# jcorsetti/oryon

Hardware: AMD Instinct MI355X
Metric: image-pairs/sec end-to-end (feat+match+reg) @224², C=256; ADD(-S) parity (higher is better)
Workload: dtype f32

## Files before the change

oryon_amd/csrc/pdsc.h:

```cpp
#pragma once
#include <stdlib.h>
#include <map>
#include <string>
#include <vector>
#include "common.h"

namespace oryon {

struct PdscLayer {
    const float *w_pcn, *b_pcn;
    const float *w_qkv, *b_qkv;
    const float *w_m1, *b_m1;
    const float *w_m2, *b_m2;
    const float *w_m3, *b_m3;
    const char *mlp_img;
    const char *mlp_img_p;
    const char *pq_img;
};

constexpr int PDSC_MLP_W1H = 0, PDSC_MLP_W1L = 16384, PDSC_MLP_W2H = 32768, PDSC_MLP_W2L = 40960, PDSC_MLP_W3H = 49152,
              PDSC_MLP_W3L = 65536, PDSC_MLP_IMG_BYTES = 81920;
constexpr int PDSC_PQ_CHUNK_BYTES = 65536, PDSC_PQ_IMG_BYTES = 5 * PDSC_PQ_CHUNK_BYTES;
constexpr int PDSC_KV_KL = 16384, PDSC_KV_VH = 32768, PDSC_KV_VL = 49152, PDSC_KV_TILE_BYTES = 65536;
constexpr int PDSC_AC_BIAS_OFF = PDSC_MLP_IMG_BYTES + 4 * 64 * (128 / 32 * 16 + 2) * 4, PDSC_AC_BIAS_BYTES = 768 * 4;
__host__ __device__ constexpr int pdsc_k_img_elem(int key, int octet) { return (octet * 64 + key) * 8; }
__host__ __device__ constexpr size_t pdsc_g4_index(int n_cap, int row, int quad) { return (size_t)quad * n_cap + row; }

struct PdscModel {
    oryon_pointdsc_config_t cfg;
    float sigma;
    float sigma_d;
    const float *w0, *b0;
    std::vector<PdscLayer> layers;
    const float *w_c1, *b_c1, *w_c2, *b_c2, *w_c3, *b_c3;
};

struct PdscWorkspace {
    float *corr_pos;
    float *feat;
    float *feat1;
    float *qkv;
    float *msg;
    char *kv_img;
    char *kv_img2;
    float *sc;
    float *att_o;
    float *att_ml;
    int att_splits;
    float *h1, *h2;
    float *feat_n;
    float *conf;
    float *seed_key;
    int32_t *seeds;
    int32_t *n_seeds;
    int32_t *knn;
    float *Mmat;
    float *seed_w;
    float *seed_dist;
    float *v_hist;
    int32_t *close_hist;
    float *seed_T;
    float *fitness;
    int32_t *best;
    float *T0;
    int S_cap, k;
};

inline int pdsc_attention_splits(int B, int n_cap)
{
    static const int forced = dev_env_int("ORYON_PDSC_ATT_SPLITS", 0);
    const int blocks = B * (n_cap / 128);
    int ks = forced ? forced : (256 + blocks - 1) / blocks;
    const int tiles = n_cap / 64;
    if (ks > 4) ks = 4;
    if (ks > tiles) ks = tiles;
    return ks < 1 ? 1 : ks;
}

inline int pdsc_seed_cap(const oryon_pointdsc_config_t &cfg, int n_cap)
{
    return (int)((double)n_cap * (double)cfg.ratio) + 1;
}

void pdsc_launch_normalise(const float *feat, int C, int n_cap, int B, const int32_t *n_rows, float *out, hipStream_t st);
int pdsc_run_encoder(const PdscModel &M, const PdscWorkspace &ws, const float *src, const float *tgt, const int32_t *n_rows,
                     int B, int n_cap, hipStream_t st);
int pdsc_run_seeds(const PdscModel &M, const float *src, const float *conf, const int32_t *n_rows, int B, int n_cap, int S_cap,
                   int32_t *seeds, int32_t *n_seeds, float *key_scratch, hipStream_t st);
int pdsc_run_hypotheses(const PdscModel &M, const PdscWorkspace &ws, const float *src, const float *tgt, const float *feat_n,
                        const int32_t *n_rows, const int32_t *seeds, const int32_t *n_seeds, int B, int n_cap, float *seed_T,
                        float *fitness, int32_t *best, float *T_best, uint8_t *labels, hipStream_t st);
int pdsc_run_refine(const PdscModel &M, const float *src, const float *tgt, const int32_t *n_rows, int B, int n_cap,
                    const float *T_in, const int32_t *status_in, const int32_t *n_seeds, float *T_out, int32_t *status_out,
                    hipStream_t st);

constexpr int PDSC_MAX_K = 64, PDSC_MAX_IT = 16;
int pdsc_run_tail(const float *src, const float *tgt, const int32_t *n_rows, const int32_t *n_seeds, int B, int n_cap, int S_cap, int k,
                  int num_iterations, float inlier_thr, const int32_t *knn, const float *Mmat, float *v_hist, int32_t *close_hist,
                  float *seed_T, float *fitness, int32_t *best, float *T_best, uint8_t *labels, hipStream_t st);
int pdsc_run_refine_tau(const float *src, const float *tgt, const int32_t *n_rows, int B, int n_cap, float tau, const float *T_in,
                        const int32_t *status_in, const int32_t *n_seeds, float *T_out, int32_t *status_out, hipStream_t st);

}
```

oryon_amd/csrc/pdsc_blocks.h:

```cpp
#pragma once
#include "common.h"
#include "pdsc.h"
#include "x3.h"

namespace oryon {

constexpr int ATT_Q = 128, ATT_KT = 64;

template <int PIECES, int WAVES, int PER_WAVE = PIECES / WAVES>
__device__ __forceinline__ void dma_pieces(const char *src, char *lds, int wave_u, int lane)
{
    static_assert(PER_WAVE * WAVES >= PIECES, "pieces per wave");
#pragma unroll
    for (int j = 0; j < PER_WAVE; ++j) {
        const int piece = wave_u * PER_WAVE + j;
        if (PER_WAVE * WAVES == PIECES || piece < PIECES)
            __builtin_amdgcn_global_load_lds((const __attribute__((address_space(1))) void *)(src + piece * 1024 + lane * 16),
                                             (__attribute__((address_space(3))) void *)(lds + piece * 1024), 16, 0, 0);
    }
}
template <int WAVES>
__device__ __forceinline__ void dma_mlp_image(const char *img, char *lds, int wave_u, int lane)
{
    dma_pieces<PDSC_MLP_IMG_BYTES / 1024, WAVES>(img, lds, wave_u, lane);
// ... 79 lines not shown
    const float *b;
    __device__ __forceinline__ float4 operator()(int off, int hi) const { return *reinterpret_cast<const float4 *>(b + off + 4 * hi); }
};
struct BiasLds {
    const float *planes;
    __device__ __forceinline__ float4 operator()(int off, int hi) const
    {
        const int q = (off >> 2) + hi;
        return make_float4(planes[q], planes[192 + q], planes[384 + q], planes[576 + q]);
    }
};

template <class Bias>
__device__ __forceinline__ void next_operand(const f32x16 (&acc)[2], const Bias &bias, int off, int hi, f16x8 (&oh)[4], f16x8 (&ol)[4])
{
#pragma unroll
    for (int rb = 0; rb < 2; ++rb)
#pragma unroll
        for (int j = 0; j < 2; ++j) {
            uint4 uh, ul;
            unsigned *ph = &uh.x, *pl = &ul.x;
#pragma unroll
            for (int g2 = 0; g2 < 2; ++g2) {
                const float4 bv = bias(off + rb * 32 + 8 * (2 * j + g2), hi);
                const int r0 = 8 * j + 4 * g2;
                const float v0 = fmaxf(acc[rb][r0] + bv.x, 0.0f), v1 = fmaxf(acc[rb][r0 + 1] + bv.y, 0.0f);
                const float v2 = fmaxf(acc[rb][r0 + 2] + bv.z, 0.0f), v3 = fmaxf(acc[rb][r0 + 3] + bv.w, 0.0f);
                split2(v0, v1, ph[2 * g2], pl[2 * g2]);
                split2(v2, v3, ph[2 * g2 + 1], pl[2 * g2 + 1]);
            }
            oh[rb * 2 + j] = __builtin_bit_cast(f16x8, uh);
            ol[rb * 2 + j] = __builtin_bit_cast(f16x8, ul);
        }
}

__device__ __forceinline__ void load_split_row(const float *row, int hi, f16x8 (&xh)[8], f16x8 (&xl)[8])
{
    const float4 *xp = reinterpret_cast<const float4 *>(row);
    float4 raw[16];
#pragma unroll
    for (int s_ = 0; s_ < 8; ++s_) { raw[2 * s_] = xp[4 * s_ + 2 * hi]; raw[2 * s_ + 1] = xp[4 * s_ + 2 * hi + 1]; }
#pragma unroll
    for (int s_ = 0; s_ < 8; ++s_) {
        uint4 uh, ul;
        split2(raw[2 * s_].x, raw[2 * s_].y, uh.x, ul.x);
        split2(raw[2 * s_].z, raw[2 * s_].w, uh.y, ul.y);
        split2(raw[2 * s_ + 1].x, raw[2 * s_ + 1].y, uh.z, ul.z);
        split2(raw[2 * s_ + 1].z, raw[2 * s_ + 1].w, uh.w, ul.w);
        xh[s_] = __builtin_bit_cast(f16x8, uh);
        xl[s_] = __builtin_bit_cast(f16x8, ul);
    }
}

__device__ __forceinline__ void att8_block_map(int &b, int &qblk)
{
    const int lin = blockIdx.x + gridDim.x * blockIdx.z;
    b = (lin / 8 / (int)gridDim.x) * 8 + (lin & 7);
    qblk = (lin / 8) % (int)gridDim.x;
}
__device__ __forceinline__ void fetch_sc(const float4 *sc_q, bool q_live, int kb, int j0, float4 (&scv)[4])
{
    const float4 *sp = sc_q + (size_t)(j0 / ATT_KT) * 8 * 64 + (size_t)kb * 4 * 64;
#pragma unroll
    for (int v4 = 0; v4 < 4; ++v4) scv[v4] = q_live ? sp[(size_t)v4 * 64] : make_float4(-1.f, -1.f, -1.f, -1.f);
}
__device__ __forceinline__ void read_k(const char *tile, int key, int s_, int hi, f16x8 (&kf)[2])
{
    kf[0] = *reinterpret_cast<const f16x8 *>(reinterpret_cast<const _Float16 *>(tile) + pdsc_k_img_elem(key, 2 * s_ + hi));
    kf[1] = *reinterpret_cast<const f16x8 *>(reinterpret_cast<const _Float16 *>(tile + PDSC_KV_KL) + pdsc_k_img_elem(key, 2 * s_ + hi));
}
__device__ __forceinline__ f16x8 read_v(const char *v_plane, int oct, int ch)
{
    return *reinterpret_cast<const f16x8 *>(reinterpret_cast<const _Float16 *>(v_plane) + ((size_t)oct * 128 + ch) * 8);
}
__device__ __forceinline__ void store_k(char *tile, float4 k, int key, int cc)
{
    uint2 uh, ul;
    split2(k.x, k.y, uh.x, ul.x);
    split2(k.z, k.w, uh.y, ul.y);
    const size_t off = (size_t)pdsc_k_img_elem(key, cc >> 3) * 2 + (cc & 7) * 2;
    *reinterpret_cast<uint2 *>(tile + off) = uh;
    *reinterpret_cast<uint2 *>(tile + PDSC_KV_KL + off) = ul;
}
__device__ __forceinline__ void store_v(char *tile, const f32x16 &acc, float bv, int kb, int ch, int hi)
{
#pragma unroll
    for (int t2 = 0; t2 < 2; ++t2) {
        uint4 uh, ul;
        split2(acc[8 * t2 + 0] + bv, acc[8 * t2 + 1] + bv, uh.x, ul.x);
        split2(acc[8 * t2 + 2] + bv, acc[8 * t2 + 3] + bv, uh.y, ul.y);
        split2(acc[8 * t2 + 4] + bv, acc[8 * t2 + 5] + bv, uh.z, ul.z);
        split2(acc[8 * t2 + 6] + bv, acc[8 * t2 + 7] + bv, uh.w, ul.w);
        const int oct = (kb * 2 + t2) * 2 + hi;
        *reinterpret_cast<uint4 *>(tile + PDSC_KV_VH + ((size_t)oct * 128 + ch) * 16) = uh;
        *reinterpret_cast<uint4 *>(tile + PDSC_KV_VL + ((size_t)oct * 128 + ch) * 16) = ul;
    }
}

}
```

oryon_amd/csrc/pdsc_encoder.hip:

```cpp
#include <stdlib.h>
#include "common.h"
#include "pdsc.h"
#include "pdsc_blocks.h"

namespace oryon {

__global__ __launch_bounds__(256) void pdsc_center_kernel(const float *__restrict__ src, const float *__restrict__ tgt,
                                                           const int32_t *__restrict__ n_rows, int n_cap,
                                                           float *__restrict__ corr_pos )
{
    __shared__ double s_part[4][6];
    __shared__ float s_mean[6];
    const int b = blockIdx.x, t = threadIdx.x, lane = t & 63, wave = t >> 6;
    const int n = n_rows[b];
    const float *s = src + (size_t)b * n_cap * 3, *g = tgt + (size_t)b * n_cap * 3;
    double acc[6] = {0, 0, 0, 0, 0, 0};
    for (int i = t; i < n; i += 256) {
#pragma unroll
        for (int d = 0; d < 3; ++d) { acc[d] += s[3 * i + d]; acc[3 + d] += g[3 * i + d]; }
    }
#pragma unroll
    for (int d = 0; d < 6; ++d) {
        double v = acc[d];
#pragma unroll
// ... 722 lines not shown
#pragma unroll
            for (int j = 0; j < 2; ++j) {
                const f16x8 bh = *reinterpret_cast<const f16x8 *>(Wh + (wn * 64 + j * 32 + l31) * XLD + ko);
                const f16x8 bl = *reinterpret_cast<const f16x8 *>(Wl + (wn * 64 + j * 32 + l31) * XLD + ko);
                acc[j] = __builtin_amdgcn_mfma_f32_32x32x16_f16(ah, bh, acc[j], 0, 0, 0);
                acc[j] = __builtin_amdgcn_mfma_f32_32x32x16_f16(ah, bl, acc[j], 0, 0, 0);
                acc[j] = __builtin_amdgcn_mfma_f32_32x32x16_f16(al, bh, acc[j], 0, 0, 0);
            }
        }
    }
#pragma unroll
    for (int j = 0; j < 2; ++j) {
        const int c = n0 + wn * 64 + j * 32 + l31;
        if (c >= N) continue;
        const float bv = bias ? bias[c] : 0.0f;
#pragma unroll
        for (int r = 0; r < 16; ++r) {
            const int row = m0 + wm * 32 + crow(r, hi);
            float v = acc[j][r] + bv;
            if (RELU) v = v > 0.0f ? v : 0.0f;
            if (RESID) v += R[(size_t)b * r_batch + (size_t)row * ldr + c];
            Y[(size_t)b * y_batch + (size_t)row * ldy + c] = v;
        }
    }
}

template <int WAVES>
__global__ __launch_bounds__(64 * WAVES) void pdsc_mlp3_x3_kernel(const float *__restrict__ msg, const float *__restrict__ resid,
                                                            const char *__restrict__ img, const float *__restrict__ b1,
                                                            const float *__restrict__ b2, const float *__restrict__ b3,
                                                            const int32_t *__restrict__ n_rows, int n_cap, float *__restrict__ out)
{
    constexpr int C = 128;
    extern __shared__ __attribute__((aligned(1024))) char mlp_lds[];
    const int b = blockIdx.y, q0 = blockIdx.x * (32 * WAVES);
    if (q0 >= n_rows[b]) return;
    const int t = threadIdx.x, lane = t & 63, wave = t >> 6, l31 = lane & 31, hi = lane >> 5;
    const int wave_u = __builtin_amdgcn_readfirstlane(wave);
    dma_mlp_image<WAVES>(img, mlp_lds, wave_u, lane);
    const size_t prow = ((size_t)b * n_cap + q0 + wave * 32 + l31) * C;
    f16x8 xh[8], xl[8];
    load_split_row(msg + prow, hi, xh, xl);
    asm volatile("s_waitcnt vmcnt(0)" ::: "memory");
    __syncthreads();
    const Frag256 w1_frag{mlp_lds, l31, hi};
    const Frag128 w23_frag{mlp_lds, l31, hi};
    f32x16 a1[2];
    two_blocks<8, false>(w1_frag, PDSC_MLP_W1H, PDSC_MLP_W1L, 0, xh, xl, a1);
    f16x8 h1h[4], h1l[4];
    next_operand(a1, BiasVector{b1}, 0, hi, h1h, h1l);
    f32x16 a2[2];
    two_blocks<4, false>(w23_frag, PDSC_MLP_W2H, PDSC_MLP_W2L, 0, h1h, h1l, a2);
    f16x8 h2h[4], h2l[4];
    next_operand(a2, BiasVector{b2}, 0, hi, h2h, h2l);
#pragma unroll
    for (int rp = 0; rp < 2; ++rp) {
        float4 rv[2][4];
#pragma unroll
        for (int i = 0; i < 2; ++i)
#pragma unroll
            for (int g = 0; g < 4; ++g) rv[i][g] = *reinterpret_cast<const float4 *>(resid + prow + (2 * rp + i) * 32 + 8 * g + 4 * hi);
        f32x16 a3[2];
        two_blocks<4, false>(w23_frag, PDSC_MLP_W3H, PDSC_MLP_W3L, 2 * rp, h2h, h2l, a3);
#pragma unroll
        for (int i = 0; i < 2; ++i)
#pragma unroll
            for (int g = 0; g < 4; ++g) {
                const int c = (2 * rp + i) * 32 + 8 * g + 4 * hi;
                const float4 bv = *reinterpret_cast<const float4 *>(b3 + c);
                float4 o;
                o.x = a3[i][4 * g + 0] + bv.x + rv[i][g].x;
                o.y = a3[i][4 * g + 1] + bv.y + rv[i][g].y;
                o.z = a3[i][4 * g + 2] + bv.z + rv[i][g].z;
                o.w = a3[i][4 * g + 3] + bv.w + rv[i][g].w;
                *reinterpret_cast<float4 *>(out + prow + c) = o;
            }
    }
}

template <int WAVES>
__global__ __launch_bounds__(64 * WAVES) void pdsc_pcn_qkv_x3_kernel(const float *__restrict__ feat, const char *__restrict__ img,
                                                               const float *__restrict__ bp, const float *__restrict__ bq,
                                                               const int32_t *__restrict__ n_rows, int n_cap, float *__restrict__ feat1,
                                                               float *__restrict__ qkv, char *__restrict__ kv_img, int g4)
{
    constexpr int C = 128, HALF = PDSC_PQ_CHUNK_BYTES / 2;
    extern __shared__ __attribute__((aligned(1024))) char pq_lds[];
    const int b = blockIdx.y, q0 = blockIdx.x * (32 * WAVES);
    if (q0 >= n_rows[b]) return;
    const int t = threadIdx.x, lane = t & 63, wave = t >> 6, l31 = lane & 31, hi = lane >> 5;
    const int wave_u = __builtin_amdgcn_readfirstlane(wave);
    dma_pq_chunk<WAVES>(img, 0, pq_lds, wave_u, lane);
    dma_pq_chunk<WAVES>(img, 1, pq_lds + PDSC_PQ_CHUNK_BYTES, wave_u, lane);
    const size_t prow = (size_t)b * n_cap + q0 + wave * 32 + l31;
    f16x8 xh[8], xl[8];
    load_split_row(feat + prow * C, hi, xh, xl);
    float bias_v[4];
#pragma unroll
    for (int i = 0; i < 4; ++i) bias_v[i] = bq[2 * C + i * 32 + l31];
    asm volatile("s_waitcnt vmcnt(0)" ::: "memory");
    asm volatile("" ::"v"(bias_v[0]), "v"(bias_v[1]), "v"(bias_v[2]), "v"(bias_v[3]));
    __syncthreads();
    const Frag256 frag{pq_lds, l31, hi};
    f16x8 fh[8], fl[8];
#pragma unroll
    for (int rp = 0; rp < 2; ++rp) {
        f32x16 acc[2];
        two_blocks<8, false>(frag, 0, HALF, 2 * rp, xh, xl, acc);
#pragma unroll
        for (int i = 0; i < 2; ++i) {
            const int rb = 2 * rp + i;
#pragma unroll
            for (int j = 0; j < 2; ++j) {
                uint4 uh, ul;
                unsigned *ph = &uh.x, *pl = &ul.x;
#pragma unroll
                for (int g2 = 0; g2 < 2; ++g2) {
                    const int c = rb * 32 + 8 * (2 * j + g2) + 4 * hi, r0 = 8 * j + 4 * g2;
                    const float4 bv = bias4(bp, rb * 32 + 8 * (2 * j + g2), hi);
                    float4 v;
                    v.x = fmaxf(acc[i][r0] + bv.x, 0.0f); v.y = fmaxf(acc[i][r0 + 1] + bv.y, 0.0f);
                    v.z = fmaxf(acc[i][r0 + 2] + bv.z, 0.0f); v.w = fmaxf(acc[i][r0 + 3] + bv.w, 0.0f);
                    if (g4) reinterpret_cast<float4 *>(feat1 + (size_t)b * n_cap * C)[pdsc_g4_index(n_cap, q0 + wave * 32 + l31, c >> 2)] = v;
                    else *reinterpret_cast<float4 *>(feat1 + prow * C + c) = v;
                    split2(v.x, v.y, ph[2 * g2], pl[2 * g2]);
                    split2(v.z, v.w, ph[2 * g2 + 1], pl[2 * g2 + 1]);
                }
                fh[rb * 2 + j] = __builtin_bit_cast(f16x8, uh);
                fl[rb * 2 + j] = __builtin_bit_cast(f16x8, ul);
            }
        }
    }
#pragma unroll
    for (int part = 0; part < 3; ++part) {
        const int area = (part + 1) & 1;
        if (part == 1) asm volatile("s_waitcnt vmcnt(16)" ::: "memory");
        if (part == 2) { if (kv_img) asm volatile("s_waitcnt vmcnt(32)" ::: "memory"); else asm volatile("s_waitcnt vmcnt(16)" ::: "memory"); }
        asm volatile("s_waitcnt lgkmcnt(0)" ::: "memory");
        __builtin_amdgcn_s_barrier();
        asm volatile("" ::: "memory");
        if (part < 2) dma_pq_chunk<WAVES>(img, part + 2, pq_lds + (area ^ 1) * PDSC_PQ_CHUNK_BYTES, wave_u, lane);
        const int p_pair = q0 + wave * 32;
        char *tile = kv_img ? kv_img + ((size_t)b * (n_cap / 64) + (p_pair >> 6)) * PDSC_KV_TILE_BYTES : nullptr;
        const bool as_v = kv_img && part == 2;
#pragma unroll
        for (int rp = 0; rp < 2; ++rp) {
            f32x16 acc[2];
            const int base_h = area * PDSC_PQ_CHUNK_BYTES;
            if (as_v) {
                two_blocks<8, true>(frag, base_h, base_h + HALF, 2 * rp, fh, fl, acc);
                const int kb = (p_pair >> 5) & 1;
#pragma unroll
                for (int i = 0; i < 2; ++i) store_v(tile, acc[i], bias_v[2 * rp + i], kb, (2 * rp + i) * 32 + l31, hi);
            } else {
                two_blocks<8, false>(frag, base_h, base_h + HALF, 2 * rp, fh, fl, acc);
#pragma unroll
                for (int i = 0; i < 2; ++i)
#pragma unroll
                    for (int g = 0; g < 4; ++g) {
                        const int cc = (2 * rp + i) * 32 + 8 * g + 4 * hi, c = part * C + cc;
                        const float4 bv = bias4(bq, part * C + (2 * rp + i) * 32 + 8 * g, hi);
                        float4 o;
                        o.x = acc[i][4 * g + 0] + bv.x; o.y = acc[i][4 * g + 1] + bv.y;
                        o.z = acc[i][4 * g + 2] + bv.z; o.w = acc[i][4 * g + 3] + bv.w;
                        if (kv_img && part == 1) {
                            store_k(tile, o, (p_pair & 63) + l31, cc);
                        } else if (g4 && part == 0) {
                            reinterpret_cast<float4 *>(qkv + (size_t)b * n_cap * 3 * C)[pdsc_g4_index(n_cap, q0 + wave * 32 + l31, cc >> 2)] = o;
                        } else {
                            *reinterpret_cast<float4 *>(qkv + prow * 3 * C + c) = o;
                        }
                    }
            }
        }
    }
}

template <int C, bool HAS_NEXT, bool DBG = false>
__global__ __launch_bounds__(512) void pdsc_att_chain_x3_kernel(const float *__restrict__ QKV, const char *__restrict__ kv_img_in,
                                                                 const float *__restrict__ sc, const int32_t *__restrict__ n_rows, int n_cap,
                                                                 float inv_sqrt_c, int n_pairs, const float *resid, const char *__restrict__ mlp_img,
                                                                 const float *__restrict__ b1, const float *__restrict__ b2,
                                                                 const float *__restrict__ b3, const char *__restrict__ pq_img,
                                                                 const float *__restrict__ bp, const float *__restrict__ bq, float *feat1,
                                                                 float *qkv, char *kv_img, float *__restrict__ feat_out, long long *dbg_clk = nullptr)
{
    constexpr int WAVES = 8, HALF = PDSC_PQ_CHUNK_BYTES / 2;
#define CLK(i) do { if constexpr (DBG) { if (blockIdx.x == 0 && blockIdx.z == 0 && (threadIdx.x & 255) == 0) dbg_clk[(threadIdx.x >> 8) * 16 + (i)] = wall_clock64(); } } while (0)
    CLK(0);
    constexpr int AREA0 = PDSC_MLP_IMG_BYTES, AREA1 = 0;
    static_assert(C == 128, "tile image geometry");
    constexpr int CB = C / 32;
    constexpr int NS = C / 16;
    extern __shared__ __attribute__((aligned(1024))) char att_lds[];
    float *lds_bias = reinterpret_cast<float *>(att_lds + PDSC_AC_BIAS_OFF);
    constexpr int SEG_B1 = 0, SEG_B2 = 64, SEG_B3 = 128, SEG_BP = 256, SEG_BQ = 384;
    const BiasLds bias4l{lds_bias};
    int b, qblk;
    att8_block_map(b, qblk);
    if (b >= n_pairs) return;
    const int n = n_rows[b];
    const int q0 = qblk * ATT_Q;
    if (q0 >= n) return;
    const int t = threadIdx.x, lane = t & 63, wave8 = t >> 6, l31 = lane & 31, hi = lane >> 5;
    const int wave_u = __builtin_amdgcn_readfirstlane(wave8);
    const int wave = wave8 & 3, kb = wave8 >> 2;
    for (int i = t; i < (HAS_NEXT ? 768 : 256); i += 512) {
        const float v = i < SEG_B2 ? b1[i] : i < SEG_B3 ? b2[i - SEG_B2] : i < SEG_BP ? b3[i - SEG_B3] : i < SEG_BQ ? bp[i - SEG_BP] : bq[i - SEG_BQ];
        lds_bias[(i & 3) * 192 + (i >> 2)] = v;
    }
    const int qrow = q0 + wave * 32 + l31;
    const float *base = QKV + (size_t)b * n_cap * 3 * C;
    const char *img = kv_img_in + (size_t)b * (n_cap / ATT_KT) * PDSC_KV_TILE_BYTES;
    const float4 *sc_q = reinterpret_cast<const float4 *>(sc) + (((size_t)b * (n_cap / 32) + (q0 / 32 + wave)) * (n_cap / ATT_KT)) * 8 * 64 + lane;
    const bool q_live = q0 + wave * 32 < n;
    float4 scv[4];
    dma_kv_tile(img, 0, att_lds, wave_u, lane);
    fetch_sc(sc_q, q_live, kb, 0, scv);
    f16x8 qh[NS], ql[NS];
    {
        const float4 *qv = reinterpret_cast<const float4 *>(base);
        const float qs = inv_sqrt_c * 1.44269504088896340736f;
#pragma unroll
        for (int s_ = 0; s_ < NS; ++s_) {
            const float4 a = qv[pdsc_g4_index(n_cap, qrow, 4 * s_ + 2 * hi)], c = qv[pdsc_g4_index(n_cap, qrow, 4 * s_ + 2 * hi + 1)];
            uint4 uh, ul;
            split2(a.x * qs, a.y * qs, uh.x, ul.x);
            split2(a.z * qs, a.w * qs, uh.y, ul.y);
            split2(c.x * qs, c.y * qs, uh.z, ul.z);
            split2(c.z * qs, c.w * qs, uh.w, ul.w);
            qh[s_] = __builtin_bit_cast(f16x8, uh);
            ql[s_] = __builtin_bit_cast(f16x8, ul);
        }
    }
    f32x16 acc_o[CB];
#pragma unroll
    for (int cb = 0; cb < CB; ++cb)
#pragma unroll
        for (int r = 0; r < 16; ++r) acc_o[cb][r] = 0.0f;
    float m_run = -INFINITY, l_run = 0.0f;

    CLK(1);
    const bool q_full = q0 + wave * 32 + 32 <= n;
    int buf = 0;
    for (int j0 = 0; j0 < n; j0 += ATT_KT, buf ^= 1) {
        asm volatile("s_waitcnt vmcnt(0)" ::: "memory");
        __syncthreads();
        if (j0 + ATT_KT < n) dma_kv_tile(img, j0 + ATT_KT, att_lds + (buf ^ 1) * PDSC_KV_TILE_BYTES, wave_u, lane);
        const char *tile = att_lds + buf * PDSC_KV_TILE_BYTES;
        f32x16 s;
#pragma unroll
        for (int r = 0; r < 16; ++r) s[r] = 0.0f;
        f16x8 kf[2][2];
        read_k(tile, kb * 32 + l31, 0, hi, kf[0]);
#pragma unroll
        for (int s_ = 0; s_ < NS; ++s_) {
            const int bf = s_ & 1;
            if (s_ + 1 < NS) read_k(tile, kb * 32 + l31, s_ + 1, hi, kf[bf ^ 1]);
            s = __builtin_amdgcn_mfma_f32_32x32x16_f16(kf[bf][0], qh[s_], s, 0, 0, 0);
            s = __builtin_amdgcn_mfma_f32_32x32x16_f16(kf[bf][0], ql[s_], s, 0, 0, 0);
            s = __builtin_amdgcn_mfma_f32_32x32x16_f16(kf[bf][1], qh[s_], s, 0, 0, 0);
        }
        float m_tile = -INFINITY;
        f16x8 ph[2], pl[2];
        if (q_full && j0 + ATT_KT <= n) {
#pragma unroll
            for (int r = 0; r < 16; ++r) {
                const float4 q4 = scv[r >> 2];
                const float scq = (r & 3) == 0 ? q4.x : (r & 3) == 1 ? q4.y : (r & 3) == 2 ? q4.z : q4.w;
                const float v = scq * s[r];
                s[r] = v;
                m_tile = fmaxf(m_tile, v);
            }
            if (j0 + ATT_KT < n) fetch_sc(sc_q, q_live, kb, j0 + ATT_KT, scv);
            m_tile = fmaxf(m_tile, __shfl_xor(m_tile, 32));
            const float m_new = fmaxf(m_run, m_tile);
            const float alpha = __builtin_amdgcn_exp2f(m_run - m_new);
            float l_tile = 0.0f;
#pragma unroll
            for (int r = 0; r < 16; r += 2) {
                const float p0 = __builtin_amdgcn_exp2f(s[r] - m_new);
                const float p1 = __builtin_amdgcn_exp2f(s[r + 1] - m_new);
                l_tile += p0;
                l_tile += p1;
                unsigned uh, ul;
                split2(p0, p1, uh, ul);
                const f16x2 h2 = __builtin_bit_cast(f16x2, uh), l2 = __builtin_bit_cast(f16x2, ul);
                ph[r >> 3][r & 7] = h2[0]; ph[r >> 3][(r & 7) + 1] = h2[1];
                pl[r >> 3][r & 7] = l2[0]; pl[r >> 3][(r & 7) + 1] = l2[1];
            }
            l_run = l_run * alpha + l_tile;
            m_run = m_new;
            if (__ballot(alpha != 1.0f) != 0ull) {
#pragma unroll
                for (int cb = 0; cb < CB; ++cb)
#pragma unroll
                    for (int r = 0; r < 16; ++r) acc_o[cb][r] *= alpha;
            }
        } else {
#pragma unroll
        for (int r = 0; r < 16; ++r) {
            const float4 q4 = scv[r >> 2];
            const float scq = (r & 3) == 0 ? q4.x : (r & 3) == 1 ? q4.y : (r & 3) == 2 ? q4.z : q4.w;
            float v = scq * s[r];
            v = (scq >= 0.0f) ? v : -INFINITY;
            s[r] = v;
            m_tile = fmaxf(m_tile, v);
        }
        if (j0 + ATT_KT < n) fetch_sc(sc_q, q_live, kb, j0 + ATT_KT, scv);
        m_tile = fmaxf(m_tile, __shfl_xor(m_tile, 32));
        const float m_new = fmaxf(m_run, m_tile);
        const float alpha = m_new == -INFINITY ? 1.0f : __builtin_amdgcn_exp2f(m_run - m_new);
        float l_tile = 0.0f;
#pragma unroll
        for (int r = 0; r < 16; r += 2) {
            const float p0 = m_new == -INFINITY ? 0.0f : __builtin_amdgcn_exp2f(s[r] - m_new);
            const float p1 = m_new == -INFINITY ? 0.0f : __builtin_amdgcn_exp2f(s[r + 1] - m_new);
            l_tile += p0;
            l_tile += p1;
            unsigned uh, ul;
            split2(p0, p1, uh, ul);
            const f16x2 h2 = __builtin_bit_cast(f16x2, uh), l2 = __builtin_bit_cast(f16x2, ul);
            ph[r >> 3][r & 7] = h2[0]; ph[r >> 3][(r & 7) + 1] = h2[1];
            pl[r >> 3][r & 7] = l2[0]; pl[r >> 3][(r & 7) + 1] = l2[1];
// ... 116 lines not shown
                    const float v2 = a3[i][4 * g + 2] + bv.z + rv[rp][i][g].z, v3 = a3[i][4 * g + 3] + bv.w + rv[rp][i][g].w;
                    split2(v0, v1, ph[2 * g2], pl[2 * g2]);
                    split2(v2, v3, ph[2 * g2 + 1], pl[2 * g2 + 1]);
                }
                xh[rb * 2 + j] = __builtin_bit_cast(f16x8, uh);
                xl[rb * 2 + j] = __builtin_bit_cast(f16x8, ul);
            }
            if constexpr (!HAS_NEXT) {
#pragma unroll
                for (int g = 0; g < 4; ++g) {
                    const int c = rb * 32 + 8 * g + 4 * hi;
                    const float4 bv = bias4l(SEG_B3 + rb * 32 + 8 * g, hi);
                    float4 o;
                    o.x = a3[i][4 * g + 0] + bv.x + rv[rp][i][g].x; o.y = a3[i][4 * g + 1] + bv.y + rv[rp][i][g].y;
                    o.z = a3[i][4 * g + 2] + bv.z + rv[rp][i][g].z; o.w = a3[i][4 * g + 3] + bv.w + rv[rp][i][g].w;
                    if (live) *reinterpret_cast<float4 *>(feat_out + prow * C + c) = o;
                }
            }
        }
    }
    }
    CLK(7);
    if constexpr (!HAS_NEXT) return;
    asm volatile("" ::"v"(bias_v[0]), "v"(bias_v[1]));
    __syncthreads();
    dma_chunk_idle(1, AREA1);
    f16x8 fh[8], fl[8];
    if (live) {
#pragma unroll
    for (int rp = 0; rp < 2; ++rp) {
        f32x16 acc[2];
        two_blocks<8, false>(frag, AREA0, AREA0 + HALF, 2 * rp, xh, xl, acc);
#pragma unroll
        for (int i = 0; i < 2; ++i) {
            const int rb = 2 * rp + i;
#pragma unroll
            for (int j = 0; j < 2; ++j) {
                uint4 uh, ul;
                unsigned *ph = &uh.x, *pl = &ul.x;
#pragma unroll
                for (int g2 = 0; g2 < 2; ++g2) {
                    const int c = rb * 32 + 8 * (2 * j + g2) + 4 * hi, r0 = 8 * j + 4 * g2;
                    const float4 bv = bias4l(SEG_BP + rb * 32 + 8 * (2 * j + g2), hi);
                    float4 v;
                    v.x = fmaxf(acc[i][r0] + bv.x, 0.0f); v.y = fmaxf(acc[i][r0 + 1] + bv.y, 0.0f);
                    v.z = fmaxf(acc[i][r0 + 2] + bv.z, 0.0f); v.w = fmaxf(acc[i][r0 + 3] + bv.w, 0.0f);
                    if (live) reinterpret_cast<float4 *>(feat1 + (size_t)b * n_cap * C)[pdsc_g4_index(n_cap, qrow, c >> 2)] = v;
                    split2(v.x, v.y, ph[2 * g2], pl[2 * g2]);
                    split2(v.z, v.w, ph[2 * g2 + 1], pl[2 * g2 + 1]);
                }
                fh[rb * 2 + j] = __builtin_bit_cast(f16x8, uh);
                fl[rb * 2 + j] = __builtin_bit_cast(f16x8, ul);
            }
        }
    }
    }
    CLK(8);
    CLK(13);
    if (kb == 1) asm volatile("s_waitcnt vmcnt(0)" ::: "memory");
    asm volatile("s_waitcnt lgkmcnt(0)" ::: "memory");
    __builtin_amdgcn_s_barrier();
    asm volatile("" ::: "memory");
    {
        f16x8 *ex = reinterpret_cast<f16x8 *>(att_lds + AREA0 + wave * 16384);
        if (live) {
#pragma unroll
            for (int f = 0; f < 8; ++f) { ex[f * 64 + lane] = fh[f]; ex[(8 + f) * 64 + lane] = fl[f]; }
        }
        asm volatile("s_waitcnt lgkmcnt(0)" ::: "memory");
        __builtin_amdgcn_s_barrier();
        asm volatile("" ::: "memory");
        if (!live) {
#pragma unroll
            for (int f = 0; f < 8; ++f) { fh[f] = ex[f * 64 + lane]; fl[f] = ex[(8 + f) * 64 + lane]; }
            asm volatile("s_waitcnt lgkmcnt(0)" ::: "memory");
        }
    }
    CLK(9);
#pragma unroll
    for (int part = 0; part < 3; ++part) {
        const int area_off = ((part + 1) & 1) ? AREA1 : AREA0, other_off = ((part + 1) & 1) ? AREA0 : AREA1;
        if (part > 0) {
            CLK(13 + part);
            if (kb == 1) { if (part == 1 || !kv_img) asm volatile("s_waitcnt vmcnt(8)" ::: "memory"); else asm volatile("s_waitcnt vmcnt(16)" ::: "memory"); }
            asm volatile("s_waitcnt lgkmcnt(0)" ::: "memory");
            __builtin_amdgcn_s_barrier();
            asm volatile("" ::: "memory");
            CLK(9 + part);
        }
        if (part < 2) dma_chunk_idle(part + 2, other_off);
        const int p_pair = q0 + wave * 32;
        char *tile = kv_img ? kv_img + ((size_t)b * (n_cap / 64) + (p_pair >> 6)) * PDSC_KV_TILE_BYTES : nullptr;
        const bool as_v = kv_img && part == 2;
        {
        const int rp = kb;
        {
            f32x16 acc[2];
            if (as_v) {
                two_blocks<8, true>(frag, area_off, area_off + HALF, 2 * rp, fh, fl, acc);
                const int kb = (p_pair >> 5) & 1;
#pragma unroll
                for (int i = 0; i < 2; ++i) store_v(tile, acc[i], bias_v[i], kb, (2 * rp + i) * 32 + l31, hi);
            } else {
                two_blocks<8, false>(frag, area_off, area_off + HALF, 2 * rp, fh, fl, acc);
#pragma unroll
                for (int i = 0; i < 2; ++i)
#pragma unroll
                    for (int g = 0; g < 4; ++g) {
                        const int cc = (2 * rp + i) * 32 + 8 * g + 4 * hi, c = part * C + cc;
                        const float4 bv = bias4l(SEG_BQ + part * C + (2 * rp + i) * 32 + 8 * g, hi);
                        float4 o;
                        o.x = acc[i][4 * g + 0] + bv.x; o.y = acc[i][4 * g + 1] + bv.y;
                        o.z = acc[i][4 * g + 2] + bv.z; o.w = acc[i][4 * g + 3] + bv.w;
                        if (kv_img && part == 1) {
                            store_k(tile, o, (p_pair & 63) + l31, cc);
                        } else if (part == 0) {
                            reinterpret_cast<float4 *>(qkv + (size_t)b * n_cap * 3 * C)[pdsc_g4_index(n_cap, qrow, cc >> 2)] = o;
                        } else {
                            *reinterpret_cast<float4 *>(qkv + prow * 3 * C + c) = o;
                        }
                    }
            }
        }
        }
    }
    CLK(12);
#undef CLK
}

__global__ __launch_bounds__(256) void pdsc_attention_merge_kernel(const float *__restrict__ part_o, const float *__restrict__ part_ml,
                                                                    const int32_t *__restrict__ n_rows, int n_cap, int C, int KS,
                                                                    int B, float *__restrict__ msg)
{
    const int b = blockIdx.y;
    const int n_live = (n_rows[b] + ATT_Q - 1) / ATT_Q * ATT_Q;
    const int c4n = C / 4;
    for (int e = blockIdx.x * blockDim.x + threadIdx.x; e < n_live * c4n; e += gridDim.x * blockDim.x) {
        const int row = e / c4n, c4 = e % c4n;
        float m = -INFINITY;
        for (int s = 0; s < KS; ++s) m = fmaxf(m, part_ml[(((size_t)s * B + b) * n_cap + row) * 2]);
        float L = 0.0f;
        float4 o = make_float4(0.f, 0.f, 0.f, 0.f);
        for (int s = 0; s < KS; ++s) {
            const size_t prow = ((size_t)s * B + b) * n_cap + row;
            const float ms = part_ml[prow * 2];
            if (ms == -INFINITY) continue;
            const float w = __expf(ms - m);
            L += w * part_ml[prow * 2 + 1];
            const float4 v = *reinterpret_cast<const float4 *>(part_o + prow * C + 4 * c4);
            o.x += w * v.x; o.y += w * v.y; o.z += w * v.z; o.w += w * v.w;
        }
        const float inv = 1.0f / L;
        o.x *= inv; o.y *= inv; o.z *= inv; o.w *= inv;
        *reinterpret_cast<float4 *>(msg + ((size_t)b * n_cap + row) * C + 4 * c4) = o;
    }
}

__global__ __launch_bounds__(256) void pdsc_normalise_kernel(const float *__restrict__ feat, int C, int n_cap,
                                                              const int32_t *__restrict__ n_rows, float *__restrict__ out)
{
    const int b = blockIdx.y;
    const int row = blockIdx.x * 4 + (threadIdx.x >> 6), lane = threadIdx.x & 63;
    if (row >= n_cap) return;
    const float *f = feat + ((size_t)b * n_cap + row) * C;
    float *o = out + ((size_t)b * n_cap + row) * C;
    float s = 0.0f;
    for (int c = lane; c < C; c += 64) s += f[c] * f[c];
#pragma unroll
    for (int off = 32; off > 0; off >>= 1) s += __shfl_xor(s, off);
    float d = sqrt_rn(s);
    d = d < 1e-12f ? 1e-12f : d;
    const bool live = row < n_rows[b];
    for (int c = lane; c < C; c += 64) o[c] = live ? f[c] / d : 0.0f;
}

constexpr int HEAD_H = 32;
__global__ __launch_bounds__(256) void pdsc_head_x3_kernel(const float *__restrict__ feat, const float *__restrict__ W1, const float *__restrict__ b1,
                                                            const float *__restrict__ W2, const float *__restrict__ b2,
                                                            const float *__restrict__ W3, const float *__restrict__ b3,
                                                            const int32_t *__restrict__ n_rows, int n_cap, float *__restrict__ conf,
                                                            float *__restrict__ feat_n)
{
    constexpr int C = 128, XLD = LIN_BK + 8;
    __shared__ __attribute__((aligned(16))) _Float16 Xh[LIN_ROWS * XLD], Xl[LIN_ROWS * XLD];
    __shared__ __attribute__((aligned(16))) _Float16 Wh[HEAD_H * XLD], Wl[HEAD_H * XLD];
    __shared__ float Hs[LIN_ROWS * HEAD_H];
    const int b = blockIdx.y, m0 = blockIdx.x * LIN_ROWS;
    const int t = threadIdx.x, lane = t & 63, wave = t >> 6, l31 = lane & 31, hi = lane >> 5;
    const int nr = n_rows[b];
    const float *x = feat + ((size_t)b * n_cap + m0) * C;
    if (m0 < nr) {
        auto layer = [&](const float *xg, int ldx, bool from_lds, const float *W, const float *bias, int K, int n_out, bool relu, bool last) {
            f32x16 acc;
#pragma unroll
            for (int r = 0; r < 16; ++r) acc[r] = 0.0f;
            for (int k0 = 0; k0 < K; k0 += LIN_BK) {
                float2 xv[4];
#pragma unroll
                for (int i = 0; i < 4; ++i) {
                    const int e = t + 256 * i, row = e >> 4, kk = (e & 15) * 2;
// ... 60 lines not shown
    }
    for (int rr = wave; rr < LIN_ROWS; rr += 4) {
        const int row = m0 + rr;
        const float *f = feat + ((size_t)b * n_cap + row) * C;
        float *o = feat_n + ((size_t)b * n_cap + row) * C;
        float s = 0.0f;
        for (int c = lane; c < C; c += 64) s += f[c] * f[c];
#pragma unroll
        for (int off = 32; off > 0; off >>= 1) s += __shfl_xor(s, off);
        float d = sqrt_rn(s);
        d = d < 1e-12f ? 1e-12f : d;
        const bool live = row < nr;
        for (int c = lane; c < C; c += 64) o[c] = live ? f[c] / d : 0.0f;
    }
}

static bool pdsc_x3()
{
    static const bool x3 = !dev_env_set("ORYON_PDSC_FP32_MFMA");
    return x3;
}

template <class... P, class... A>
static void launch_lds(void (*kernel)(P...), dim3 grid, dim3 block, int lds, hipStream_t st, A... args)
{
    allow_dynamic_lds(reinterpret_cast<const void *>(kernel), lds);
    hipLaunchKernelGGL(kernel, grid, block, lds, st, args...);
}

static int launch_linear(bool relu, bool resid, const float *X, int ldx, size_t xb, const float *W, const float *bias,
                         const float *R, int ldr, size_t rb, float *Y, int ldy, size_t yb, int K, int N, int B, int n_cap,
                         const int32_t *n_rows, hipStream_t st)
{
    using Kernel = decltype(&pdsc_linear_kernel<false, false>);
    static const Kernel table[2][2][2] = {
        {{pdsc_linear_kernel<false, false>, pdsc_linear_kernel<false, true>}, {pdsc_linear_kernel<true, false>, pdsc_linear_kernel<true, true>}},
        {{pdsc_linear_x3_kernel<false, false>, pdsc_linear_x3_kernel<false, true>}, {pdsc_linear_x3_kernel<true, false>, pdsc_linear_x3_kernel<true, true>}}};
    const bool x3 = pdsc_x3() && K % LIN_BK == 0 && ldx % 2 == 0;
    hipLaunchKernelGGL(table[x3][relu][resid], dim3(n_cap / LIN_ROWS, ceil_div(N, LIN_COLS), B), dim3(256), 0, st, X, ldx, xb, W, bias, R, ldr, rb,
                       Y, ldy, yb, K, N, n_rows);
    return hipGetLastError() == hipSuccess ? ORYON_OK : ORYON_ERR_HIP;
}

void pdsc_launch_normalise(const float *feat, int C, int n_cap, int B, const int32_t *n_rows, float *out, hipStream_t st)
{
    hipLaunchKernelGGL(pdsc_normalise_kernel, dim3(n_cap / 4, B), dim3(256), 0, st, feat, C, n_cap, n_rows, out);
}

enum class PdscRoute { plain, fused, chain };
struct PdscPlan {
    PdscRoute route;
    bool x3;
    int waves;
    bool img;
};
static PdscPlan plan_encoder(const PdscModel &M, const PdscWorkspace &ws, int n_cap)
{
    static const int forced = dev_env_int("ORYON_PDSC_ROUTE", 0);
    PdscPlan p = {PdscRoute::plain, pdsc_x3(), n_cap % 256 == 0 ? 8 : 4, ws.att_splits == 1 && ws.kv_img != nullptr};
    bool images = true;
    for (const PdscLayer &L : M.layers) images = images && L.mlp_img && L.mlp_img_p && L.pq_img;
    if (M.cfg.num_channels != 128 || !p.x3 || !images || forced == 1) return p;
    p.route = (p.waves == 8 && p.img && ws.kv_img2 && forced != 2) ? PdscRoute::chain : PdscRoute::fused;
    return p;
}

int pdsc_run_encoder(const PdscModel &M, const PdscWorkspace &ws, const float *src, const float *tgt, const int32_t *n_rows,
                     int B, int n_cap, hipStream_t st)
{
    const int C = M.cfg.num_channels, H = C / 2;
    const size_t fb = (size_t)n_cap * C, qb = (size_t)n_cap * 3 * C, hb = (size_t)n_cap * H;
    hipLaunchKernelGGL(pdsc_center_kernel, dim3(B), dim3(256), 0, st, src, tgt, n_rows, n_cap, ws.corr_pos);
    int rc = launch_linear(false, false, ws.corr_pos, 8, (size_t)n_cap * 8, M.w0, M.b0, nullptr, 0, 0, ws.feat, C, fb, M.cfg.in_dim, C,
                           B, n_cap, n_rows, st);
    if (rc) return rc;
    const float inv_sigma2 = 1.0f / (M.sigma_d * M.sigma_d);
    const float inv_sqrt_c = 1.0f / sqrtf((float)C);
    hipLaunchKernelGGL(pdsc_sc_kernel, dim3(n_cap / 128, n_cap / ATT_KT, B), dim3(256), 0, st, src, tgt, n_rows, n_cap, inv_sigma2, ws.sc);

    const PdscPlan plan = plan_encoder(M, ws, n_cap);
    const dim3 att8_grid(n_cap / ATT_Q, 1, (B + 7) / 8 * 8);
    auto pcn_qkv = [&](const PdscLayer &L, int waves, char *kv_img, int g4) {
        launch_lds(waves == 8 ? pdsc_pcn_qkv_x3_kernel<8> : pdsc_pcn_qkv_x3_kernel<4>, dim3(n_cap / (32 * waves), B), dim3(64 * waves),
                   2 * PDSC_PQ_CHUNK_BYTES, st, ws.feat, L.pq_img, L.b_pcn, L.b_qkv, n_rows, n_cap, ws.feat1, ws.qkv, kv_img, g4);
    };
    auto attention = [&]() {
        const int KS = ws.att_splits;
        const auto kernel = (C == 128 && plan.x3) ? pdsc_attention_x3_kernel<128> : C == 128 ? pdsc_attention_kernel<128>
                            : C == 64             ? pdsc_attention_kernel<64> : pdsc_attention_kernel<32>;
        hipLaunchKernelGGL(kernel, dim3(n_cap / ATT_Q, KS, B), dim3(256), 0, st, ws.qkv, ws.sc, n_rows, n_cap, inv_sqrt_c, ws.msg, KS, ws.att_o, ws.att_ml);
        if (KS > 1)
            hipLaunchKernelGGL(pdsc_attention_merge_kernel, dim3((n_cap * (C / 4) + 255) / 256, B), dim3(256), 0, st, ws.att_o, ws.att_ml,
                               n_rows, n_cap, C, KS, B, ws.msg);
    };
    for (int l = 0; l < M.cfg.num_layers; ++l) {
        const PdscLayer &L = M.layers[l];
        switch (plan.route) {
        case PdscRoute::chain: {
            constexpr int AC_LDS = PDSC_AC_BIAS_OFF + PDSC_AC_BIAS_BYTES;
            static_assert(PDSC_AC_BIAS_OFF >= 2 * PDSC_KV_TILE_BYTES && AC_LDS <= 160 * 1024, "att_chain LDS budget");
            char *kv_cur = (l & 1) ? ws.kv_img2 : ws.kv_img, *kv_nxt = (l & 1) ? ws.kv_img : ws.kv_img2;
            if (l == 0) pcn_qkv(L, 8, ws.kv_img, 1);
            const bool has_next = l + 1 < M.cfg.num_layers;
            const PdscLayer &N = M.layers[has_next ? l + 1 : l];
#ifdef ORYON_DEV
            static const int clocks = dev_env_int("ORYON_PDSC_CLOCKS", 0);
            if (clocks > 0 && l == clocks && has_next) {
                static long long *dclk = nullptr;
                if (!dclk) { (void)hipMalloc(reinterpret_cast<void **>(&dclk), 32 * sizeof(long long)); }
                (void)hipMemsetAsync(dclk, 0, 32 * sizeof(long long), st);
                launch_lds(pdsc_att_chain_x3_kernel<128, true, true>, att8_grid, dim3(512), AC_LDS, st, ws.qkv, kv_cur, ws.sc, n_rows, n_cap, inv_sqrt_c, B,
                           ws.feat1, L.mlp_img_p, L.b_m1, L.b_m2, L.b_m3, N.pq_img, N.b_pcn, N.b_qkv, ws.feat1, ws.qkv, kv_nxt, ws.feat, dclk);
                long long hc[32];
                (void)hipMemcpyAsync(hc, dclk, sizeof(hc), hipMemcpyDeviceToHost, st);
                (void)hipStreamSynchronize(st);
                fprintf(stderr, "att_chain clocks (us since entry) wave0:");
                for (int i = 1; i <= 15; ++i) fprintf(stderr, " %.2f", hc[i] ? (hc[i] - hc[0]) * 0.01 : -1.0);
                fprintf(stderr, "  wave4:");
                for (int i = 1; i <= 12; ++i) fprintf(stderr, " %.2f", hc[16 + i] ? (hc[16 + i] - hc[16]) * 0.01 : -1.0);
                fprintf(stderr, "\n");
                continue;
            }
#endif
            if (has_next)
                launch_lds(pdsc_att_chain_x3_kernel<128, true>, att8_grid, dim3(512), AC_LDS, st, ws.qkv, kv_cur, ws.sc, n_rows, n_cap, inv_sqrt_c, B,
                           ws.feat1, L.mlp_img_p, L.b_m1, L.b_m2, L.b_m3, N.pq_img, N.b_pcn, N.b_qkv, ws.feat1, ws.qkv, kv_nxt, ws.feat, nullptr);
            else
                launch_lds(pdsc_att_chain_x3_kernel<128, false>, att8_grid, dim3(512), AC_LDS, st, ws.qkv, kv_cur, ws.sc, n_rows, n_cap, inv_sqrt_c, B,
                           ws.feat1, L.mlp_img_p, L.b_m1, L.b_m2, L.b_m3, nullptr, nullptr, nullptr, ws.feat1, ws.qkv, kv_nxt, ws.feat, nullptr);
            break;
        }
        case PdscRoute::fused:
            pcn_qkv(L, plan.waves, plan.img ? ws.kv_img : nullptr, 0);
            if (plan.img)
                launch_lds(pdsc_attention_x3_img8_kernel<128>, att8_grid, dim3(512), 2 * PDSC_KV_TILE_BYTES, st, ws.qkv, ws.kv_img, ws.sc, n_rows, n_cap,
                           inv_sqrt_c, ws.msg, B);
            else
                attention();
            launch_lds(plan.waves == 8 ? pdsc_mlp3_x3_kernel<8> : pdsc_mlp3_x3_kernel<4>, dim3(n_cap / (32 * plan.waves), B), dim3(64 * plan.waves),
                       PDSC_MLP_IMG_BYTES, st, ws.msg, ws.feat1, L.mlp_img, L.b_m1, L.b_m2, L.b_m3, n_rows, n_cap, ws.feat);
            break;
        case PdscRoute::plain:
            rc = launch_linear(true, false, ws.feat, C, fb, L.w_pcn, L.b_pcn, nullptr, 0, 0, ws.feat1, C, fb, C, C, B, n_cap, n_rows, st);
            if (rc) return rc;
            rc = launch_linear(false, false, ws.feat1, C, fb, L.w_qkv, L.b_qkv, nullptr, 0, 0, ws.qkv, 3 * C, qb, C, 3 * C, B, n_cap, n_rows, st);
            if (rc) return rc;
            attention();
            rc = launch_linear(true, false, ws.msg, C, fb, L.w_m1, L.b_m1, nullptr, 0, 0, ws.h1, H, hb, C, H, B, n_cap, n_rows, st);
            if (rc) return rc;
            rc = launch_linear(true, false, ws.h1, H, hb, L.w_m2, L.b_m2, nullptr, 0, 0, ws.h2, H, hb, H, H, B, n_cap, n_rows, st);
            if (rc) return rc;
            rc = launch_linear(false, true, ws.h2, H, hb, L.w_m3, L.b_m3, ws.feat1, C, fb, ws.feat, C, fb, H, C, B, n_cap, n_rows, st);
            if (rc) return rc;
            break;
        }
        if (hipGetLastError() != hipSuccess) return ORYON_ERR_HIP;
    }
    static const bool fused_head = dev_env_int("ORYON_PDSC_FUSED_HEAD", 1) != 0;
    if (fused_head && C == 128 && n_cap % LIN_ROWS == 0) {
        hipLaunchKernelGGL(pdsc_head_x3_kernel, dim3(n_cap / LIN_ROWS, B), dim3(256), 0, st, ws.feat, M.w_c1, M.b_c1, M.w_c2, M.b_c2, M.w_c3, M.b_c3,
                           n_rows, n_cap, ws.conf, ws.feat_n);
        return hipGetLastError() == hipSuccess ? ORYON_OK : ORYON_ERR_HIP;
    }
    rc = launch_linear(true, false, ws.feat, C, fb, M.w_c1, M.b_c1, nullptr, 0, 0, ws.h1, 32, (size_t)n_cap * 32, C, 32, B, n_cap, n_rows, st);
    if (rc) return rc;
    rc = launch_linear(true, false, ws.h1, 32, (size_t)n_cap * 32, M.w_c2, M.b_c2, nullptr, 0, 0, ws.h2, 32, (size_t)n_cap * 32, 32, 32, B, n_cap, n_rows, st);
    if (rc) return rc;
// ... 8 lines not shown
```

Before: 23840.

## Store Q pre-scaled and pre-split to f16 hi/lo in MFMA fragment layout

The QKV producer kernels now write Q already multiplied by the softmax scale and split into f16 high/low planes, laid out by k-step and half so the attention kernel loads ready-made MFMA fragments as uint4. This removes the per-attention-block fp32 load, scaling and split work and halves the register conversion cost in the attention prologue. It also reorders the bias staging and score fetch in the attention prologue, and adjusts the vmcnt waits and scheduling barriers around the chunk DMAs to account for the changed number of outstanding stores. The attention path now depends on the producer having written this layout, and the changed wait counts could be wrong if the store counts differ.

Result: no change. 24100 (median of 2 runs) (+1.1%).

```diff
diff --git a/oryon_amd/csrc/pdsc.h b/oryon_amd/csrc/pdsc.h
--- a/oryon_amd/csrc/pdsc.h
+++ b/oryon_amd/csrc/pdsc.h
@@ -25,6 +25,13 @@
 constexpr int PDSC_AC_BIAS_OFF = PDSC_MLP_IMG_BYTES + 4 * 64 * (128 / 32 * 16 + 2) * 4, PDSC_AC_BIAS_BYTES = 768 * 4;
 __host__ __device__ constexpr int pdsc_k_img_elem(int key, int octet) { return (octet * 64 + key) * 8; }
 __host__ __device__ constexpr size_t pdsc_g4_index(int n_cap, int row, int quad) { return (size_t)quad * n_cap + row; }
+__host__ __device__ constexpr size_t pdsc_qs_block(int n_cap, int kstep, int plane) { return (size_t)(plane * 8 + kstep) * 2 * n_cap; }
+__host__ __device__ constexpr unsigned pdsc_qs_slot(int n_cap, int row, int half) { return (unsigned)(half * n_cap + row); }
+__host__ __device__ constexpr size_t pdsc_qs_index(int n_cap, int row, int kstep, int half, int plane)
+{
+    return pdsc_qs_block(n_cap, kstep, plane) + pdsc_qs_slot(n_cap, row, half);
+}
+__host__ __device__ inline float pdsc_q_scale(float inv_sqrt_c) { return inv_sqrt_c * 1.44269504088896340736f; }
 
 struct PdscModel {
     oryon_pointdsc_config_t cfg;
diff --git a/oryon_amd/csrc/pdsc_blocks.h b/oryon_amd/csrc/pdsc_blocks.h
--- a/oryon_amd/csrc/pdsc_blocks.h
+++ b/oryon_amd/csrc/pdsc_blocks.h
@@ -185,6 +185,15 @@
     *reinterpret_cast<uint2 *>(tile + off) = uh;
     *reinterpret_cast<uint2 *>(tile + PDSC_KV_KL + off) = ul;
 }
+__device__ __forceinline__ void store_qs(float *q_pair, int n_cap, int row, int rb, int g, int hi, const float4 o, float qs)
+{
+    uint2 uh, ul;
+    split2(o.x * qs, o.y * qs, uh.x, ul.x);
+    split2(o.z * qs, o.w * qs, uh.y, ul.y);
+    char *p = reinterpret_cast<char *>(q_pair) + hi * 8;
+    *reinterpret_cast<uint2 *>(p + pdsc_qs_index(n_cap, row, 2 * rb + (g >> 1), g & 1, 0) * 16) = uh;
+    *reinterpret_cast<uint2 *>(p + pdsc_qs_index(n_cap, row, 2 * rb + (g >> 1), g & 1, 1) * 16) = ul;
+}
 __device__ __forceinline__ void store_v(char *tile, const f32x16 &acc, float bv, int kb, int ch, int hi)
 {
 #pragma unroll
diff --git a/oryon_amd/csrc/pdsc_encoder.hip b/oryon_amd/csrc/pdsc_encoder.hip
--- a/oryon_amd/csrc/pdsc_encoder.hip
+++ b/oryon_amd/csrc/pdsc_encoder.hip
@@ -828,7 +828,7 @@
 __global__ __launch_bounds__(64 * WAVES) void pdsc_pcn_qkv_x3_kernel(const float *__restrict__ feat, const char *__restrict__ img,
                                                                const float *__restrict__ bp, const float *__restrict__ bq,
                                                                const int32_t *__restrict__ n_rows, int n_cap, float *__restrict__ feat1,
-                                                               float *__restrict__ qkv, char *__restrict__ kv_img, int g4)
+                                                               float *__restrict__ qkv, char *__restrict__ kv_img, int g4, float inv_sqrt_c)
 {
     constexpr int C = 128, HALF = PDSC_PQ_CHUNK_BYTES / 2;
     extern __shared__ __attribute__((aligned(1024))) char pq_lds[];
@@ -880,12 +880,16 @@
 #pragma unroll
     for (int part = 0; part < 3; ++part) {
         const int area = (part + 1) & 1;
-        if (part == 1) asm volatile("s_waitcnt vmcnt(16)" ::: "memory");
+        if (part == 1) { if (g4) asm volatile("s_waitcnt vmcnt(32)" ::: "memory"); else asm volatile("s_waitcnt vmcnt(16)" ::: "memory"); }
         if (part == 2) { if (kv_img) asm volatile("s_waitcnt vmcnt(32)" ::: "memory"); else asm volatile("s_waitcnt vmcnt(16)" ::: "memory"); }
         asm volatile("s_waitcnt lgkmcnt(0)" ::: "memory");
         __builtin_amdgcn_s_barrier();
         asm volatile("" ::: "memory");
-        if (part < 2) dma_pq_chunk<WAVES>(img, part + 2, pq_lds + (area ^ 1) * PDSC_PQ_CHUNK_BYTES, wave_u, lane);
+        if (part < 2) {
+            dma_pq_chunk<WAVES>(img, part + 2, pq_lds + (area ^ 1) * PDSC_PQ_CHUNK_BYTES, wave_u, lane);
+            __builtin_amdgcn_sched_barrier(0);
+            asm volatile("" ::: "memory");
+        }
         const int p_pair = q0 + wave * 32;
         char *tile = kv_img ? kv_img + ((size_t)b * (n_cap / 64) + (p_pair >> 6)) * PDSC_KV_TILE_BYTES : nullptr;
         const bool as_v = kv_img && part == 2;
@@ -912,7 +916,7 @@
                         if (kv_img && part == 1) {
                             store_k(tile, o, (p_pair & 63) + l31, cc);
                         } else if (g4 && part == 0) {
-                            reinterpret_cast<float4 *>(qkv + (size_t)b * n_cap * 3 * C)[pdsc_g4_index(n_cap, q0 + wave * 32 + l31, cc >> 2)] = o;
+                            store_qs(qkv + (size_t)b * n_cap * 3 * C, n_cap, q0 + wave * 32 + l31, 2 * rp + i, g, hi, o, pdsc_q_scale(inv_sqrt_c));
                         } else {
                             *reinterpret_cast<float4 *>(qkv + prow * 3 * C + c) = o;
                         }
@@ -951,10 +955,6 @@
     const int t = threadIdx.x, lane = t & 63, wave8 = t >> 6, l31 = lane & 31, hi = lane >> 5;
     const int wave_u = __builtin_amdgcn_readfirstlane(wave8);
     const int wave = wave8 & 3, kb = wave8 >> 2;
-    for (int i = t; i < (HAS_NEXT ? 768 : 256); i += 512) {
-        const float v = i < SEG_B2 ? b1[i] : i < SEG_B3 ? b2[i - SEG_B2] : i < SEG_BP ? b3[i - SEG_B3] : i < SEG_BQ ? bp[i - SEG_BP] : bq[i - SEG_BQ];
-        lds_bias[(i & 3) * 192 + (i >> 2)] = v;
-    }
     const int qrow = q0 + wave * 32 + l31;
     const float *base = QKV + (size_t)b * n_cap * 3 * C;
     const char *img = kv_img_in + (size_t)b * (n_cap / ATT_KT) * PDSC_KV_TILE_BYTES;
@@ -962,22 +962,29 @@
     const bool q_live = q0 + wave * 32 < n;
     float4 scv[4];
     dma_kv_tile(img, 0, att_lds, wave_u, lane);
-    fetch_sc(sc_q, q_live, kb, 0, scv);
     f16x8 qh[NS], ql[NS];
     {
-        const float4 *qv = reinterpret_cast<const float4 *>(base);
-        const float qs = inv_sqrt_c * 1.44269504088896340736f;
+        static_assert(NS == 8, "QS layout: 8 k-steps");
+        const uint4 *qv = reinterpret_cast<const uint4 *>(base);
+        const unsigned slot = pdsc_qs_slot(n_cap, qrow, hi);
 #pragma unroll
         for (int s_ = 0; s_ < NS; ++s_) {
-            const float4 a = qv[pdsc_g4_index(n_cap, qrow, 4 * s_ + 2 * hi)], c = qv[pdsc_g4_index(n_cap, qrow, 4 * s_ + 2 * hi + 1)];
-            uint4 uh, ul;
-            split2(a.x * qs, a.y * qs, uh.x, ul.x);
-            split2(a.z * qs, a.w * qs, uh.y, ul.y);
-            split2(c.x * qs, c.y * qs, uh.z, ul.z);
-            split2(c.z * qs, c.w * qs, uh.w, ul.w);
-            qh[s_] = __builtin_bit_cast(f16x8, uh);
-            ql[s_] = __builtin_bit_cast(f16x8, ul);
-        }
+            qh[s_] = __builtin_bit_cast(f16x8, (qv + pdsc_qs_block(n_cap, s_, 0))[slot]);
+            ql[s_] = __builtin_bit_cast(f16x8, (qv + pdsc_qs_block(n_cap, s_, 1))[slot]);
+        }
+    }
+    constexpr int NB = HAS_NEXT ? 768 : 256;
+    float bias_in[2] = {0.0f, 0.0f};
+#pragma unroll
+    for (int k = 0; k < 2; ++k) {
+        const int i = t + 512 * k;
+        if (i < NB) bias_in[k] = i < SEG_B2 ? b1[i] : i < SEG_B3 ? b2[i - SEG_B2] : i < SEG_BP ? b3[i - SEG_B3] : i < SEG_BQ ? bp[i - SEG_BP] : bq[i - SEG_BQ];
+    }
+    fetch_sc(sc_q, q_live, kb, 0, scv);
+#pragma unroll
+    for (int k = 0; k < 2; ++k) {
+        const int i = t + 512 * k;
+        if (i < NB) lds_bias[(i & 3) * 192 + (i >> 2)] = bias_in[k];
     }
     f32x16 acc_o[CB];
 #pragma unroll
@@ -986,6 +993,7 @@
         for (int r = 0; r < 16; ++r) acc_o[cb][r] = 0.0f;
     float m_run = -INFINITY, l_run = 0.0f;
 
+    if constexpr (DBG) asm volatile("s_waitcnt vmcnt(0)" ::: "memory");
     CLK(1);
     const bool q_full = q0 + wave * 32 + 32 <= n;
     int buf = 0;
@@ -1268,13 +1276,17 @@
         const int area_off = ((part + 1) & 1) ? AREA1 : AREA0, other_off = ((part + 1) & 1) ? AREA0 : AREA1;
         if (part > 0) {
             CLK(13 + part);
-            if (kb == 1) { if (part == 1 || !kv_img) asm volatile("s_waitcnt vmcnt(8)" ::: "memory"); else asm volatile("s_waitcnt vmcnt(16)" ::: "memory"); }
+            if (kb == 1) { if (part == 1 || kv_img) asm volatile("s_waitcnt vmcnt(16)" ::: "memory"); else asm volatile("s_waitcnt vmcnt(8)" ::: "memory"); }
             asm volatile("s_waitcnt lgkmcnt(0)" ::: "memory");
             __builtin_amdgcn_s_barrier();
             asm volatile("" ::: "memory");
             CLK(9 + part);
         }
-        if (part < 2) dma_chunk_idle(part + 2, other_off);
+        if (part < 2) {
+            dma_chunk_idle(part + 2, other_off);
+            __builtin_amdgcn_sched_barrier(0);
+            asm volatile("" ::: "memory");
+        }
         const int p_pair = q0 + wave * 32;
         char *tile = kv_img ? kv_img + ((size_t)b * (n_cap / 64) + (p_pair >> 6)) * PDSC_KV_TILE_BYTES : nullptr;
         const bool as_v = kv_img && part == 2;
@@ -1301,7 +1313,7 @@
                         if (kv_img && part == 1) {
                             store_k(tile, o, (p_pair & 63) + l31, cc);
                         } else if (part == 0) {
-                            reinterpret_cast<float4 *>(qkv + (size_t)b * n_cap * 3 * C)[pdsc_g4_index(n_cap, qrow, cc >> 2)] = o;
+                            store_qs(qkv + (size_t)b * n_cap * 3 * C, n_cap, qrow, 2 * rp + i, g, hi, o, pdsc_q_scale(inv_sqrt_c));
                         } else {
                             *reinterpret_cast<float4 *>(qkv + prow * 3 * C + c) = o;
                         }
@@ -1528,7 +1540,7 @@
     const dim3 att8_grid(n_cap / ATT_Q, 1, (B + 7) / 8 * 8);
     auto pcn_qkv = [&](const PdscLayer &L, int waves, char *kv_img, int g4) {
         launch_lds(waves == 8 ? pdsc_pcn_qkv_x3_kernel<8> : pdsc_pcn_qkv_x3_kernel<4>, dim3(n_cap / (32 * waves), B), dim3(64 * waves),
-                   2 * PDSC_PQ_CHUNK_BYTES, st, ws.feat, L.pq_img, L.b_pcn, L.b_qkv, n_rows, n_cap, ws.feat1, ws.qkv, kv_img, g4);
+                   2 * PDSC_PQ_CHUNK_BYTES, st, ws.feat, L.pq_img, L.b_pcn, L.b_qkv, n_rows, n_cap, ws.feat1, ws.qkv, kv_img, g4, inv_sqrt_c);
     };
     auto attention = [&]() {
         const int KS = ws.att_splits;
```
